# MarSaKi/ETPNav

Measured on AMD Instinct MI355X. Metric: planner fwd+bwd steps/sec at batch 32, 36-view x768 pano + 80-tok instr, higher is better.
Workload: dtype bf16

## Files before the change

### etpnav_amd/csrc/attn_rows.hip

```cpp
#include <stdlib.h>
#include <string.h>

#include "kernels.h"

namespace etp {
namespace {

constexpr int TQ = 128;
constexpr int TP = 144;
constexpr int PROJ_K = 768;
constexpr int PROJ_SLAB_K = 128;
constexpr int PROJ_RING = 3;
#ifndef ETP_PROJ_FETCH_AT
#define ETP_PROJ_FETCH_AT 2
#endif
__device__ __forceinline__ int tile_off(int row, int chunk) { return row * TQ + ((chunk ^ (row & 7)) << 4); }

struct RowArgs {
  const bf16_t *Q, *K, *V; long ldq, ldk, ldv;
  float* lse;
  bf16_t* ctx; long ldc;
  int nh, Lq, Lk;
  Drop drop;
  const uint8_t* keymask; int mask_mode; const float* dist; const float* sp_w; const float* sp_b;
  float alpha;
  const bf16_t* dO; long ldd;
  bf16_t *dQ, *dK, *dV; long lddq, lddk, lddv;
  float *d_sp_w, *d_sp_b;
  const bf16_t* W; long ldw; int Kp;
  const bf16_t* X; long ldx; const float* bqkv;
  int kv_mod;
};

__device__ __forceinline__ f32x4_t mma32(const uint4& a, const uint4& b, f32x4_t c) {
  return __builtin_amdgcn_mfma_f32_16x16x32_bf16(__builtin_bit_cast(bf16x8_t, a), __builtin_bit_cast(bf16x8_t, b), c, 0, 0, 0);
}
__device__ __forceinline__ f32x4_t mma16(const short4_t& a, const short4_t& b, f32x4_t c) {
  return __builtin_amdgcn_mfma_f32_16x16x16bf16_1k(a, b, c, 0, 0, 0);
}
__device__ __forceinline__ short4_t pack4(float a, float b, float c, float d) {
  const uint2 u = make_uint2(pack_bf16(a, b), pack_bf16(c, d));
  return __builtin_bit_cast(short4_t, u);
}
__device__ __forceinline__ uint4 frag(const char* tile, int row0, int s, int lane) {
  return *reinterpret_cast<const uint4*>(tile + tile_off(row0 + (lane & 15), s * 4 + (lane >> 4)));
}
__device__ __forceinline__ short4_t frag_t4(const char* tile, int row0, int col0, int lane) {
  const int i = lane & 15, g = lane >> 4;
  const int col = col0 + (i & 3) * 4;
  const char* p = tile + tile_off(row0 + 4 * g + (i >> 2), col >> 3) + (col & 7) * 2;
  typedef short4_t __attribute__((address_space(3))) * lds_s4;
  return __builtin_amdgcn_ds_read_tr16_b64_v4i16((lds_s4)(p));
}

template <int MAXROWS> struct TileRegs {
  static constexpr int N = (MAXROWS * 8 + 255) / 256;
  uint4 v[N];
};
template <int MAXROWS>
__device__ __forceinline__ void tile_fetch(TileRegs<MAXROWS>& r, const bf16_t* __restrict__ g, long ld, int rows_valid, int rows_pad,
                                           int tid, int nthr) {
#pragma unroll
  for (int j = 0; j < TileRegs<MAXROWS>::N; ++j) {
    const int q = tid + j * nthr, row = q >> 3, c = (q & 7) * 8;
    uint4 v = make_uint4(0u, 0u, 0u, 0u);
    if (row < rows_pad) {
      const bool ok = row < rows_valid;
      v = *reinterpret_cast<const uint4*>(g + (long)min(row, rows_valid - 1) * ld + c);
      v.x = ok ? v.x : 0u; v.y = ok ? v.y : 0u; v.z = ok ? v.z : 0u; v.w = ok ? v.w : 0u;
    }
    r.v[j] = v;
  }
}
template <int MAXROWS>
__device__ __forceinline__ void tile_commit(char* lds, const TileRegs<MAXROWS>& r, int rows_pad, int tid, int nthr) {
#pragma unroll
  for (int j = 0; j < TileRegs<MAXROWS>::N; ++j) {
    const int q = tid + j * nthr, row = q >> 3;
    if (row < rows_pad) *reinterpret_cast<uint4*>(lds + tile_off(row, q & 7)) = r.v[j];
  }
}

__device__ __forceinline__ void store_rows16(char* strip, const f32x4_t (&acc)[4], float scale, bf16_t* __restrict__ g0, long ld,
                                             int rows_valid, int lane) {
  const int i = lane & 15, g = lane >> 4;
#pragma unroll
  for (int t = 0; t < 4; ++t)
    *reinterpret_cast<uint2*>(strip + i * TP + (16 * t + 4 * g) * 2) =
        make_uint2(pack_bf16(acc[t][0] * scale, acc[t][1] * scale), pack_bf16(acc[t][2] * scale, acc[t][3] * scale));
  __builtin_amdgcn_wave_barrier();
#pragma unroll
  for (int j = 0; j < 2; ++j) {
    const int c = lane + 64 * j, row = c >> 3, part = c & 7;
    const uint4 v = *reinterpret_cast<const uint4*>(strip + row * TP + part * 16);
    if (row < rows_valid) *reinterpret_cast<uint4*>(g0 + (long)row * ld + part * 8) = v;
  }
  __builtin_amdgcn_wave_barrier();
}

template <int WN>
__device__ __forceinline__ void proj_load_w(uint4 (&w)[WN], const bf16_t* __restrict__ Wg, long ldw, int s, int tid, int nthr) {
#pragma unroll
  for (int j = 0; j < WN; ++j) {
    const int p = tid + j * nthr;
    w[j] = make_uint4(0u, 0u, 0u, 0u);
    if (p < PROJ_SLAB_K * 8) w[j] = *reinterpret_cast<const uint4*>(Wg + (long)(s * PROJ_SLAB_K + (p >> 3)) * ldw + (p & 7) * 8);
  }
}
__device__ __forceinline__ void proj_load_y(uint4 (&y)[4], const bf16_t* __restrict__ Yr, int s, bool computing, bool qok) {
#pragma unroll
  for (int u = 0; u < 4; ++u) {
    uint4 v = make_uint4(0u, 0u, 0u, 0u);
    if (computing) v = *reinterpret_cast<const uint4*>(Yr + s * PROJ_SLAB_K + 32 * u);
    v.x = qok ? v.x : 0u; v.y = qok ? v.y : 0u; v.z = qok ? v.z : 0u; v.w = qok ? v.w : 0u;
    y[u] = v;
  }
}
template <int WN>
__device__ __forceinline__ void proj_commit_w(char* slab, const uint4 (&w)[WN], int tid, int nthr) {
#pragma unroll
  for (int j = 0; j < WN; ++j) {
    const int p = tid + j * nthr, kk = p >> 3;
    const int row = (kk & ~0x1c) | ((kk & 0x4) << 2) | ((kk & 0x18) >> 1);
    if (p < PROJ_SLAB_K * 8) *reinterpret_cast<uint4*>(slab + tile_off(row, p & 7)) = w[j];
  }
}

template <int WN>
__device__ __forceinline__ void qkv_load_w(uint4 (&w)[WN], const bf16_t* __restrict__ W, long ldw, int Hh, int h, int s, int tid, int nthr) {
#pragma unroll
  for (int j = 0; j < WN; ++j) {
    const int p = tid + j * nthr, row = p >> 3;
    w[j] = make_uint4(0u, 0u, 0u, 0u);
    if (p < 192 * 8) w[j] = *reinterpret_cast<const uint4*>(W + (long)((row >> 6) * Hh + h * 64 + (row & 63)) * ldw + s * 64 + (p & 7) * 8);
  }
}
__device__ __forceinline__ void qkv_load_x(uint4 (&y)[2], const bf16_t* __restrict__ Xr, int s, bool computing, bool ok) {
#pragma unroll
  for (int u = 0; u < 2; ++u) {
    uint4 v = make_uint4(0u, 0u, 0u, 0u);
    if (computing) v = *reinterpret_cast<const uint4*>(Xr + s * 64 + 32 * u);
    v.x = ok ? v.x : 0u; v.y = ok ? v.y : 0u; v.z = ok ? v.z : 0u; v.w = ok ? v.w : 0u;
    y[u] = v;
  }
}
template <int WN>
__device__ __forceinline__ void qkv_commit_w(char* slab, const uint4 (&w)[WN], int tid, int nthr) {
#pragma unroll
  for (int j = 0; j < WN; ++j) {
    const int p = tid + j * nthr;
    if (p < 192 * 8) *reinterpret_cast<uint4*>(slab + tile_off(p >> 3, p & 7)) = w[j];
  }
}

__device__ __forceinline__ float key_term(const uint8_t* km, int col, int Lk, int mask_mode) {
  if (col >= Lk) return -INFINITY;
  if (km && !km[col]) return mask_mode ? -INFINITY : -10000.0f;
  return 0.f;
}

constexpr int QKV_SLAB_K = 64;
constexpr int QKV_RING = 2;
constexpr int QKV_SLAB_BYTES = 192 * TQ;
__host__ __device__ constexpr int rows_fwd_bias_off(int BKV, int nwaves) {
  const int base = 2 * BKV * TQ + BKV * 4 + nwaves * 16 * TP, ring = QKV_RING * QKV_SLAB_BYTES;
  return base < ring ? ring : base;
}
__host__ __device__ constexpr int rows_fwd_lds(int BKV, int nwaves, bool qkv) {
  return qkv ? rows_fwd_bias_off(BKV, nwaves) + 192 * 4 : 2 * BKV * TQ + BKV * 4 + nwaves * 16 * TP;
}

template <int NKT, bool HAS_DIST, bool QKV>
__global__ __launch_bounds__(512) void rows_fwd_kernel(const RowArgs a) {
  constexpr int BKV = NKT * 16;
  extern __shared__ __attribute__((aligned(16))) char smem[];
  char* kt = smem; char* vt = smem + BKV * TQ;
  float* kadd = reinterpret_cast<float*>(smem + 2 * BKV * TQ);
  const int tid = threadIdx.x, nthr = blockDim.x, lane = tid & 63, wave = tid >> 6, i = lane & 15, g = lane >> 4;
  const int bh = blockIdx.x, b = bh / a.nh, h = bh % a.nh;
  char* strip = smem + 2 * BKV * TQ + BKV * 4 + wave * 16 * TP;
  const int q = wave * 16 + i, qc = min(q, a.Lq - 1);
  uint4 qf0, qf1;

  const int bk = a.kv_mod > 0 ? b % a.kv_mod : b;
  if constexpr (!QKV) {
    TileRegs<BKV> rk, rv;
    tile_fetch<BKV>(rk, a.K + (long)bk * a.Lk * a.ldk + h * 64, a.ldk, a.Lk, BKV, tid, nthr);
    tile_fetch<BKV>(rv, a.V + (long)bk * a.Lk * a.ldv + h * 64, a.ldv, a.Lk, BKV, tid, nthr);
    const bf16_t* Qr = a.Q + ((long)b * a.Lq + qc) * a.ldq + h * 64 + g * 8;
    qf0 = *reinterpret_cast<const uint4*>(Qr); qf1 = *reinterpret_cast<const uint4*>(Qr + 32);
    if (tid < BKV) kadd[tid] = key_term(a.keymask ? a.keymask + (long)bk * a.Lk : nullptr, tid, a.Lk, a.mask_mode);
    tile_commit<BKV>(kt, rk, BKV, tid, nthr);
    tile_commit<BKV>(vt, rv, BKV, tid, nthr);
  } else {
    constexpr int NS = PROJ_K / QKV_SLAB_K, WN = 6;
    const int Hh = a.nh * 64;
    float* bias_l = reinterpret_cast<float*>(smem + rows_fwd_bias_off(BKV, nthr >> 6));
    const bool computing = wave < NKT, tok_ok = q < a.Lq;
    const bf16_t* Xr = a.X + ((long)b * a.Lq + qc) * a.ldx + g * 8;
    uint4 wr[WN], yb[2][2];
    f32x4_t acc[12];
#pragma unroll
    for (int t = 0; t < 12; ++t) acc[t] = f32x4_t{0.f, 0.f, 0.f, 0.f};
    if (tid < 192) bias_l[tid] = a.bqkv ? a.bqkv[(tid >> 6) * Hh + h * 64 + (tid & 63)] : 0.f;
    qkv_load_w<WN>(wr, a.W, a.ldw, Hh, h, 0, tid, nthr); qkv_load_x(yb[0], Xr, 0, computing, tok_ok);
    qkv_commit_w<WN>(smem, wr, tid, nthr);
    __syncthreads();
#pragma unroll
    for (int s = 0; s < NS; ++s) {
      if (s + 1 < NS) { qkv_load_w<WN>(wr, a.W, a.ldw, Hh, h, s + 1, tid, nthr); qkv_load_x(yb[(s + 1) & 1], Xr, s + 1, computing, tok_ok); }
      if (computing) {
        const char* slab = smem + (s & 1) * QKV_SLAB_BYTES;
#pragma unroll
        for (int u = 0; u < 2; ++u)
#pragma unroll
          for (int t = 0; t < 12; ++t) acc[t] = mma32(frag(slab, 16 * t, u, lane), yb[s & 1][u], acc[t]);
      }
      if (s + 1 < NS) qkv_commit_w<WN>(smem + ((s + 1) & 1) * QKV_SLAB_BYTES, wr, tid, nthr);
      __syncthreads();
    }
    if (tid < BKV) kadd[tid] = key_term(a.keymask ? a.keymask + (long)b * a.Lk : nullptr, tid, a.Lk, a.mask_mode);
    if (computing) {
      const int rows_valid = a.Lq - wave * 16;
#pragma unroll
      for (int sec = 0; sec < 3; ++sec) {
#pragma unroll
        for (int t = 0; t < 4; ++t) {
          const float4 bb = *reinterpret_cast<const float4*>(bias_l + sec * 64 + 16 * t + 4 * g);
          const f32x4_t c = acc[sec * 4 + t];
          *reinterpret_cast<uint2*>(strip + i * TP + (16 * t + 4 * g) * 2) =
              make_uint2(pack_bf16(c[0] + bb.x, c[1] + bb.y), pack_bf16(c[2] + bb.z, c[3] + bb.w));
        }
        __builtin_amdgcn_wave_barrier();
        if (sec == 0) {
          qf0 = *reinterpret_cast<const uint4*>(strip + i * TP + g * 16);
          qf1 = *reinterpret_cast<const uint4*>(strip + i * TP + 64 + g * 16);
        }
        bf16_t* dst = const_cast<bf16_t*>(sec == 0 ? a.Q : sec == 1 ? a.K : a.V);
        const long ld = sec == 0 ? a.ldq : sec == 1 ? a.ldk : a.ldv;
        char* tile = sec == 1 ? kt : vt;
#pragma unroll
        for (int j = 0; j < 2; ++j) {
          const int c = lane + 64 * j, row = c >> 3, part = c & 7;
          uint4 v = *reinterpret_cast<const uint4*>(strip + row * TP + part * 16);
          if (row < rows_valid) *reinterpret_cast<uint4*>(dst + ((long)b * a.Lq + wave * 16 + row) * ld + h * 64 + part * 8) = v;
          else v = make_uint4(0u, 0u, 0u, 0u);
          if (sec > 0) *reinterpret_cast<uint4*>(tile + tile_off(wave * 16 + row, part)) = v;
        }
        __builtin_amdgcn_wave_barrier();
      }
    }
  }
  __syncthreads();
  if (wave * 16 >= a.Lq) return;

  f32x4_t s[NKT];
#pragma unroll
  for (int n = 0; n < NKT; ++n) {
    s[n] = f32x4_t{0.f, 0.f, 0.f, 0.f};
    s[n] = mma32(frag(kt, 16 * n, 0, lane), qf0, s[n]);
    s[n] = mma32(frag(kt, 16 * n, 1, lane), qf1, s[n]);
  }
  float w = 0.f, b0 = 0.f;
  const float* drow = nullptr;
  if constexpr (HAS_DIST) { w = a.sp_w[0]; b0 = a.sp_b[0]; drow = a.dist + ((long)b * a.Lq + qc) * a.Lk; }
  float mx = -INFINITY;
#pragma unroll
  for (int n = 0; n < NKT; ++n) {
    const float4 ka4 = *reinterpret_cast<const float4*>(kadd + 16 * n + 4 * g);
    const float ka[4] = {ka4.x, ka4.y, ka4.z, ka4.w};
#pragma unroll
    for (int r = 0; r < 4; ++r) {
      float v = s[n][r] * a.alpha + ka[r];
      if constexpr (HAS_DIST) {
        const int key = 16 * n + 4 * g + r;
        if (key < a.Lk) v += w * drow[key] + b0;
      }
      s[n][r] = v;
      mx = fmaxf(mx, v);
    }
  }
  mx = fmaxf(mx, __shfl_xor(mx, 16, 64));
  mx = fmaxf(mx, __shfl_xor(mx, 32, 64));
  float sum = 0.f;
#pragma unroll
  for (int n = 0; n < NKT; ++n)
#pragma unroll
    for (int r = 0; r < 4; ++r) {
      const float e = __expf(s[n][r] - mx);
      s[n][r] = e;
      sum += e;
    }
  sum += __shfl_xor(sum, 16, 64);
  sum += __shfl_xor(sum, 32, 64);
  const float inv = 1.0f / sum;
  if (g == 0 && q < a.Lq) a.lse[(long)bh * a.Lq + q] = mx + __logf(sum);

  short4_t pb[NKT];
  const bool dropping = a.drop.p > 0.f;
  const uint32_t rbase = ((uint32_t)bh * a.Lq + q) * (uint32_t)a.Lk;
#pragma unroll
  for (int n = 0; n < NKT; ++n) {
    float p[4];
#pragma unroll
    for (int r = 0; r < 4; ++r) p[r] = s[n][r] * inv;
    if (dropping) {
      float dm[4];
      drop_mult_run<4>(a.drop.seed, rbase + 16 * n + 4 * g, a.drop.p, a.drop.inv_keep, dm);
#pragma unroll
      for (int r = 0; r < 4; ++r) p[r] *= dm[r];
    }
    pb[n] = pack4(p[0], p[1], p[2], p[3]);
  }
  f32x4_t o[4];
#pragma unroll
  for (int t = 0; t < 4; ++t) o[t] = f32x4_t{0.f, 0.f, 0.f, 0.f};
#pragma unroll
  for (int n = 0; n < NKT; ++n)
#pragma unroll
    for (int t = 0; t < 4; ++t) o[t] = mma16(frag_t4(vt, 16 * n, 16 * t, lane), pb[n], o[t]);
  store_rows16(strip, o, 1.0f, a.ctx + ((long)b * a.Lq + wave * 16) * a.ldc + h * 64, a.ldc, a.Lq - wave * 16, lane);
}

struct BwdLds {
  int q, d, k, v, kadd, lse, D, red, strip, ring, total;
  __host__ __device__ BwdLds(int BQ, int BKV, bool proj = false) {
    d = 0; q = BQ * TQ; k = 2 * BQ * TQ; v = k + BKV * TQ; kadd = v + BKV * TQ;
    lse = kadd + BKV * 4; D = lse + 128 * 4; red = D + 128 * 4; strip = red + 16 * 4; total = strip + 8 * 16 * TP;
    ring = BQ * TQ;
    if (proj && total < ring + PROJ_RING * PROJ_SLAB_K * TQ) total = ring + PROJ_RING * PROJ_SLAB_K * TQ;
  }
};

template <int NKT, bool HAS_DIST, bool PROJ>
__global__ __launch_bounds__(512) void rows_bwd_kernel(const RowArgs a) {
  constexpr int BKV = NKT * 16;
  extern __shared__ __attribute__((aligned(16))) char smem[];
  const int nqt = (a.Lq + 15) >> 4, BQ = nqt * 16;
  const BwdLds L(BQ, BKV, PROJ);
  char *qt = smem + L.q, *dt = smem + L.d, *kt = smem + L.k, *vt = smem + L.v;
  float* kadd = reinterpret_cast<float*>(smem + L.kadd);
  float* lse = reinterpret_cast<float*>(smem + L.lse);
  float* Dl = reinterpret_cast<float*>(smem + L.D);
  float* red = reinterpret_cast<float*>(smem + L.red);
  const int tid = threadIdx.x, nthr = blockDim.x, lane = tid & 63, wave = tid >> 6, i = lane & 15, g = lane >> 4;
  const int bh = blockIdx.x, b = bh / a.nh, h = bh % a.nh;
  const bool dropping = a.drop.p > 0.f;
  char* strip = smem + L.strip + wave * 16 * TP;

  {
    TileRegs<128> rq, rd;
    TileRegs<BKV> rk, rv;
    const int bk = a.kv_mod > 0 ? b % a.kv_mod : b;
#define FETCH_QKV()                                                                                        \
    tile_fetch<128>(rq, a.Q + (long)b * a.Lq * a.ldq + h * 64, a.ldq, a.Lq, BQ, tid, nthr);                 \
    tile_fetch<BKV>(rk, a.K + (long)bk * a.Lk * a.ldk + h * 64, a.ldk, a.Lk, BKV, tid, nthr);               \
    tile_fetch<BKV>(rv, a.V + (long)bk * a.Lk * a.ldv + h * 64, a.ldv, a.Lk, BKV, tid, nthr)
    if constexpr (!PROJ) {
      FETCH_QKV();
      tile_fetch<128>(rd, a.dO + (long)b * a.Lq * a.ldd + h * 64, a.ldd, a.Lq, BQ, tid, nthr);
    } else {
      constexpr int SLAB = PROJ_SLAB_K * TQ, WN = 4, NS = PROJ_K / PROJ_SLAB_K;
      char* ring = smem + L.ring;
      const bf16_t* Wg = a.W + h * 64;
      const int qrow = wave * 16 + i;
      const bool computing = wave < nqt, qok = qrow < a.Lq;
      const bf16_t* Yr = a.dO + ((long)b * a.Lq + min(qrow, a.Lq - 1)) * a.ldd + g * 8;
      uint4 wr[2][WN], yb[3][4];
      f32x4_t acc[4];
#pragma unroll
      for (int t = 0; t < 4; ++t) acc[t] = f32x4_t{0.f, 0.f, 0.f, 0.f};
      proj_load_w<WN>(wr[0], Wg, a.ldw, 0, tid, nthr); proj_load_y(yb[0], Yr, 0, computing, qok);
      proj_load_w<WN>(wr[1], Wg, a.ldw, 1, tid, nthr); proj_load_y(yb[1], Yr, 1, computing, qok);
      proj_commit_w<WN>(ring, wr[0], tid, nthr);
      __syncthreads();
#pragma unroll
      for (int s = 0; s < NS; ++s) {
        if (s + 2 < NS) { proj_load_w<WN>(wr[s % 2], Wg, a.ldw, s + 2, tid, nthr); proj_load_y(yb[(s + 2) % 3], Yr, s + 2, computing, qok); }
        if (s + ETP_PROJ_FETCH_AT == NS) { FETCH_QKV(); }
        if (computing) {
          const char* slab = ring + (s % 3) * SLAB;
#pragma unroll
          for (int u = 0; u < 4; ++u)
#pragma unroll
            for (int t = 0; t < 4; ++t) {
              const short4_t lo = frag_t4(slab, 32 * u, 16 * t, lane), hi = frag_t4(slab, 32 * u + 16, 16 * t, lane);
              const uint2 l2 = __builtin_bit_cast(uint2, lo), h2 = __builtin_bit_cast(uint2, hi);
              acc[t] = mma32(make_uint4(l2.x, l2.y, h2.x, h2.y), yb[s % 3][u], acc[t]);
            }
        }
        if (s + 1 < NS) {
          proj_commit_w<WN>(ring + ((s + 1) % 3) * SLAB, wr[(s + 1) % 2], tid, nthr);
          __syncthreads();
        }
      }
      if (computing) {
#pragma unroll
        for (int t = 0; t < 4; ++t)
          *reinterpret_cast<uint2*>(dt + tile_off(16 * wave + i, 2 * t + (g >> 1)) + (g & 1) * 8) =
              make_uint2(pack_bf16(acc[t][0], acc[t][1]), pack_bf16(acc[t][2], acc[t][3]));
      }
      __syncthreads();
    }
#undef FETCH_QKV
    if (tid < BKV) kadd[tid] = key_term(a.keymask ? a.keymask + (long)bk * a.Lk : nullptr, tid, a.Lk, a.mask_mode);
    if (tid < 128) lse[tid] = tid < a.Lq ? a.lse[(long)bh * a.Lq + tid] : INFINITY;
    tile_commit<128>(qt, rq, BQ, tid, nthr);
    if constexpr (!PROJ) tile_commit<128>(dt, rd, BQ, tid, nthr);
    tile_commit<BKV>(kt, rk, BKV, tid, nthr);
    tile_commit<BKV>(vt, rv, BKV, tid, nthr);
  }
  float w = 0.f, b0 = 0.f;
  if constexpr (HAS_DIST) { w = a.sp_w[0]; b0 = a.sp_b[0]; }
  __syncthreads();

  float aw = 0.f, ab = 0.f;
  if (wave < nqt) {
    const int q = wave * 16 + i;
    const bool qok = q < a.Lq;
    const uint4 qf0 = frag(qt, 16 * wave, 0, lane), qf1 = frag(qt, 16 * wave, 1, lane);
    const uint4 df0 = frag(dt, 16 * wave, 0, lane), df1 = frag(dt, 16 * wave, 1, lane);
    const float lse_i = lse[q];
    const float* drow = HAS_DIST ? a.dist + ((long)b * a.Lq + min(q, a.Lq - 1)) * a.Lk : nullptr;
    const uint32_t rbase = ((uint32_t)bh * a.Lq + q) * (uint32_t)a.Lk;
    f32x4_t p[NKT], dp[NKT];
    float dv4[NKT][4];
    float Dp = 0.f;
#pragma unroll
    for (int n = 0; n < NKT; ++n) {
      f32x4_t st = f32x4_t{0.f, 0.f, 0.f, 0.f}, dpt = f32x4_t{0.f, 0.f, 0.f, 0.f};
      st = mma32(frag(kt, 16 * n, 0, lane), qf0, st);
      st = mma32(frag(kt, 16 * n, 1, lane), qf1, st);
      dpt = mma32(frag(vt, 16 * n, 0, lane), df0, dpt);
      dpt = mma32(frag(vt, 16 * n, 1, lane), df1, dpt);
      const float4 ka4 = *reinterpret_cast<const float4*>(kadd + 16 * n + 4 * g);
      const float ka[4] = {ka4.x, ka4.y, ka4.z, ka4.w};
      float dm[4] = {1.f, 1.f, 1.f, 1.f};
      if (dropping) drop_mult_run<4>(a.drop.seed, rbase + 16 * n + 4 * g, a.drop.p, a.drop.inv_keep, dm);
#pragma unroll
      for (int r = 0; r < 4; ++r) {
        const int key = 16 * n + 4 * g + r;
        float v = st[r] * a.alpha + ka[r];
        if constexpr (HAS_DIST) {
          const float dd = (qok && key < a.Lk) ? drow[key] : 0.f;
          dv4[n][r] = dd;
          if (key < a.Lk) v += w * dd + b0;
        }
        const float pe = __expf(v - lse_i);
        const float dpv = dpt[r] * dm[r];
        p[n][r] = pe; dp[n][r] = dpv;
        Dp += pe * dpv;
      }
    }
    Dp += __shfl_xor(Dp, 16, 64);
    Dp += __shfl_xor(Dp, 32, 64);
    if (g == 0) Dl[q] = Dp;
    short4_t dsb[NKT];
#pragma unroll
    for (int n = 0; n < NKT; ++n) {
      float ds[4];
#pragma unroll
      for (int r = 0; r < 4; ++r) {
        ds[r] = p[n][r] * (dp[n][r] - Dp);
        if constexpr (HAS_DIST) { aw += ds[r] * dv4[n][r]; ab += ds[r]; }
      }
      dsb[n] = pack4(ds[0], ds[1], ds[2], ds[3]);
    }
    f32x4_t dq[4];
#pragma unroll
    for (int t = 0; t < 4; ++t) dq[t] = f32x4_t{0.f, 0.f, 0.f, 0.f};
#pragma unroll
    for (int n = 0; n < NKT; ++n)
#pragma unroll
      for (int t = 0; t < 4; ++t) dq[t] = mma16(frag_t4(kt, 16 * n, 16 * t, lane), dsb[n], dq[t]);
    store_rows16(strip, dq, a.alpha, a.dQ + ((long)b * a.Lq + wave * 16) * a.lddq + h * 64, a.lddq, a.Lq - wave * 16, lane);
  }
  if constexpr (HAS_DIST) {
    aw = wave_sum(aw); ab = wave_sum(ab);
    if (lane == 0) { red[wave] = aw; red[8 + wave] = ab; }
  }
  __syncthreads();
  if constexpr (HAS_DIST) {
    if (tid == 0 && a.d_sp_w != nullptr) {
      float sw = 0.f, sb = 0.f;
      for (int k = 0; k < (nthr >> 6); ++k) { sw += red[k]; sb += red[8 + k]; }
      atomicAdd(a.d_sp_w, sw);
      atomicAdd(a.d_sp_b, sb);
    }
  }

  if (wave * 16 < a.Lk) {
    const int key = wave * 16 + i;
    const bool kok = key < a.Lk;
    const uint4 kf0 = frag(kt, 16 * wave, 0, lane), kf1 = frag(kt, 16 * wave, 1, lane);
    const uint4 vf0 = frag(vt, 16 * wave, 0, lane), vf1 = frag(vt, 16 * wave, 1, lane);
    const float ka = kadd[key];
    f32x4_t dv[4], dk[4];
#pragma unroll
    for (int t = 0; t < 4; ++t) { dv[t] = f32x4_t{0.f, 0.f, 0.f, 0.f}; dk[t] = f32x4_t{0.f, 0.f, 0.f, 0.f}; }
    for (int m = 0; m < nqt; ++m) {
      f32x4_t s = f32x4_t{0.f, 0.f, 0.f, 0.f}, dpm = f32x4_t{0.f, 0.f, 0.f, 0.f};
      s = mma32(frag(qt, 16 * m, 0, lane), kf0, s);
      s = mma32(frag(qt, 16 * m, 1, lane), kf1, s);
      dpm = mma32(frag(dt, 16 * m, 0, lane), vf0, dpm);
      dpm = mma32(frag(dt, 16 * m, 1, lane), vf1, dpm);
      const float4 l4 = *reinterpret_cast<const float4*>(lse + 16 * m + 4 * g);
      const float4 D4 = *reinterpret_cast<const float4*>(Dl + 16 * m + 4 * g);
      const float lr[4] = {l4.x, l4.y, l4.z, l4.w}, Dr[4] = {D4.x, D4.y, D4.z, D4.w};
      float pd[4], ds[4];
#pragma unroll
      for (int r = 0; r < 4; ++r) {
        const int qq = 16 * m + 4 * g + r;
        float v = s[r] * a.alpha + ka;
        if constexpr (HAS_DIST) {
          if (kok && qq < a.Lq) v += w * a.dist[((long)b * a.Lq + qq) * a.Lk + key] + b0;
        }
        const float pe = __expf(v - lr[r]);
        float mult = 1.0f;
        if (dropping) mult = drop_mult(a.drop.seed, ((uint32_t)bh * a.Lq + qq) * (uint32_t)a.Lk + key, a.drop.p, a.drop.inv_keep);
        pd[r] = pe * mult;
        ds[r] = pe * (dpm[r] * mult - Dr[r]);
      }
      const short4_t pb = pack4(pd[0], pd[1], pd[2], pd[3]), dsb = pack4(ds[0], ds[1], ds[2], ds[3]);
#pragma unroll
      for (int t = 0; t < 4; ++t) {
        dv[t] = mma16(frag_t4(dt, 16 * m, 16 * t, lane), pb, dv[t]);
        dk[t] = mma16(frag_t4(qt, 16 * m, 16 * t, lane), dsb, dk[t]);
      }
    }
    store_rows16(strip, dv, 1.0f, a.dV + ((long)b * a.Lk + wave * 16) * a.lddv + h * 64, a.lddv, a.Lk - wave * 16, lane);
    store_rows16(strip, dk, a.alpha, a.dK + ((long)b * a.Lk + wave * 16) * a.lddk + h * 64, a.lddk, a.Lk - wave * 16, lane);
  }
}

template <int NKT, bool HAS_DIST, bool QKV> int launch_rows_fwd_q(const RowArgs& k, int blocks, int threads, hipStream_t st) {
  const int smem = rows_fwd_lds(NKT * 16, threads / 64, QKV);
  auto kern = rows_fwd_kernel<NKT, HAS_DIST, QKV>;
  if (smem > 64 * 1024) ETP_CHECK_HIP(ensure_dyn_lds(reinterpret_cast<const void*>(kern), smem));
  ETP_LAUNCH_ROW(ROWF_ATTN_FWD, kern, dim3(blocks), dim3(threads), smem, st, k);
  ETP_CHECK_LAUNCH(QKV ? "attn_rows_fwd_qkv" : "attn_rows_fwd");
  return ETP_OK;
}
template <int NKT, bool HAS_DIST> int launch_rows_fwd(const RowArgs& k, int blocks, int threads, hipStream_t st) {
  return k.X ? launch_rows_fwd_q<NKT, HAS_DIST, true>(k, blocks, threads, st) : launch_rows_fwd_q<NKT, HAS_DIST, false>(k, blocks, threads, st);
}
template <int NKT, bool HAS_DIST, bool PROJ> int launch_rows_bwd_p(const RowArgs& k, int blocks, int threads, hipStream_t st) {
  const BwdLds L(((k.Lq + 15) >> 4) * 16, NKT * 16, PROJ);
  auto kern = rows_bwd_kernel<NKT, HAS_DIST, PROJ>;
  ETP_CHECK_HIP(ensure_dyn_lds(reinterpret_cast<const void*>(kern), BwdLds(128, NKT * 16, PROJ).total));
  ETP_LAUNCH_ROW(ROWF_ATTN_BWD, kern, dim3(blocks), dim3(threads), L.total, st, k);
  ETP_CHECK_LAUNCH(PROJ ? "attn_rows_bwd_proj" : "attn_rows_bwd");
  return ETP_OK;
}
template <int NKT, bool HAS_DIST> int launch_rows_bwd(const RowArgs& k, int blocks, int threads, hipStream_t st) {
  return k.W ? launch_rows_bwd_p<NKT, HAS_DIST, true>(k, blocks, threads, st) : launch_rows_bwd_p<NKT, HAS_DIST, false>(k, blocks, threads, st);
}

template <bool HAS_DIST> int dispatch_fwd(int nkt, const RowArgs& k, int blocks, int threads, hipStream_t st) {
  switch (nkt) {
    case 1: return launch_rows_fwd<1, HAS_DIST>(k, blocks, threads, st);
    case 2: return launch_rows_fwd<2, HAS_DIST>(k, blocks, threads, st);
    case 3: return launch_rows_fwd<3, HAS_DIST>(k, blocks, threads, st);
    case 4: return launch_rows_fwd<4, HAS_DIST>(k, blocks, threads, st);
    case 5: return launch_rows_fwd<5, HAS_DIST>(k, blocks, threads, st);
    case 6: return launch_rows_fwd<6, HAS_DIST>(k, blocks, threads, st);
    case 7: return launch_rows_fwd<7, HAS_DIST>(k, blocks, threads, st);
    default: return launch_rows_fwd<8, HAS_DIST>(k, blocks, threads, st);
  }
}
template <bool HAS_DIST> int dispatch_bwd(int nkt, const RowArgs& k, int blocks, int threads, hipStream_t st) {
  switch (nkt) {
    case 1: return launch_rows_bwd<1, HAS_DIST>(k, blocks, threads, st);
    case 2: return launch_rows_bwd<2, HAS_DIST>(k, blocks, threads, st);
    case 3: return launch_rows_bwd<3, HAS_DIST>(k, blocks, threads, st);
    case 4: return launch_rows_bwd<4, HAS_DIST>(k, blocks, threads, st);
    case 5: return launch_rows_bwd<5, HAS_DIST>(k, blocks, threads, st);
    case 6: return launch_rows_bwd<6, HAS_DIST>(k, blocks, threads, st);
    case 7: return launch_rows_bwd<7, HAS_DIST>(k, blocks, threads, st);
    default: return launch_rows_bwd<8, HAS_DIST>(k, blocks, threads, st);
  }
}

RowArgs make_row_args(int nh, const AttnBuf& a, void* P, float alpha, Drop drop) {
  RowArgs k;
  memset(&k, 0, sizeof(k));
  k.Q = (const bf16_t*)a.Q; k.K = (const bf16_t*)a.K; k.V = (const bf16_t*)a.V; k.ldq = a.ldq; k.ldk = a.ldk; k.ldv = a.ldv;
  k.lse = (float*)P; k.nh = nh; k.Lq = a.Lq; k.Lk = a.Lk; k.drop = drop;
  k.keymask = a.keymask; k.mask_mode = a.mask_mode; k.dist = a.dist; k.sp_w = a.sp_w; k.sp_b = a.sp_b; k.alpha = alpha;
  k.kv_mod = a.kv_mod;
  return k;
}

}

bool attn_rows_ok(int dt, const AttnBuf& a, long ldc) {
  const bool on = opt_on(OPT_ATTN_ROWS, true);
  if (!on || dt != ETP_BF16) return false;
  if (a.Lq > 128 || a.Lk > 128 || a.Lq < 1 || a.Lk < 1 || a.ldS < 2) return false;
// ... 62 lines not shown
```

### etpnav_amd/csrc/planner.hip

```cpp
#include <string.h>

#include <algorithm>
#include <functional>
#include <vector>

#include "kernels.h"

namespace etp {

struct AttnP { int qkv_w, qkv_b, o_w, o_b, ln_g, ln_b; };
struct FfnP { int i_w, i_b, o_w, o_b, ln_g, ln_b; };
struct TxtLayerP { AttnP att; FfnP ffn; };
struct PanoLayerP { int in_w, in_b, out_w, out_b, l1_w, l1_b, l2_w, l2_b, n1_g, n1_b, n2_g, n2_b; };
struct XLayerP { int q_w, q_b, kv_w, kv_b, xo_w, xo_b, xln_g, xln_b; AttnP self; FfnP ffn;
                 AttnP lself; FfnP lffn; };

struct PInfo { std::string name; int ndim; long shape[2]; int region; long offset; long numel; };

}

struct etp_planner {
  etp_config cfg;
  std::vector<etp::PInfo> params;
  long total = 0, n_matrix = 0;
// ... 388 lines not shown
  g.M = a.Lq; g.N = a.Lk; g.K = dh; g.nb_inner = nh; g.alpha = alpha;
  ETP_TRY(launch_gemm(dt, dt, 0, 0, g, a.B * nh, st));
  ETP_TRY(softmax_fwd(dt, P, a.keymask, a.dist, a.sp_w, a.sp_b, a.B, nh, a.Lq, a.Lk, a.ldS, a.mask_mode, st));
  const void* Pv = P;
  if (drop.p > 0.f) {
    ETP_TRY(drop_rows(dt, P, a.Pd, (long)a.B * nh * a.Lq, a.Lk, a.ldS, drop, st));
    Pv = a.Pd;
  }
  GemmArgs h = base_args();
  h.A = Pv; h.lda = a.ldS; h.sAo = g.sCo; h.sAi = g.sCi;
  h.B = a.V; h.ldb = a.ldv; h.sBo = (long)a.Lk * a.ldv; h.sBi = dh;
  h.C = ctx; h.ldc = ldc; h.sCo = (long)a.Lq * ldc; h.sCi = dh;
  h.M = a.Lq; h.N = dh; h.K = a.Lk; h.nb_inner = nh;
  return launch_gemm(dt, dt, 0, 1, h, a.B * nh, st);
}

int attn_bwd_impl(int dt, int nh, const AttnBuf& a, const void* P, const void* dctx, long ldd, void* dP, void* dQ, long lddq,
                  void* dK, long lddk, void* dV, long lddv, float alpha, float* d_sp_w, float* d_sp_b, hipStream_t st,
                  Drop drop) {
  const int dh = 64;
  ETP_REQUIRE(!a.dkv_sum || a.kv_mod > 0, "summed dK/dV (AttnBuf::dkv_sum) needs per-episode K/V indirection (kv_mod > 0)");
  {
    const int epc = dt == ETP_BF16 ? 8 : 4;
    const long ldc_f = a.O != nullptr ? a.ldo : ldd;
    const bool dal = lddq % epc == 0 && lddk % epc == 0 && lddv % epc == 0;
    const int fam = attn_family(dt, a, ldc_f);
    if (fam == ATTN_FAMILY_ROWS) {
      ETP_REQUIRE(ldd % 8 == 0 && dal, "the forward of this shape kept lse only (register-resident kernels): the backward needs "
                                       "16-byte-aligned dctx / dQ / dK / dV rows");
      return attn_rows_bwd(nh, a, P, dctx, ldd, dQ, lddq, dK, lddk, dV, lddv, alpha, d_sp_w, d_sp_b, st, drop);
    }
    ETP_REQUIRE(a.kv_mod == 0 || fam == ATTN_FAMILY_FLASH, "per-episode K/V indirection (AttnBuf::kv_mod) needs the register-resident or the streaming attention kernels (bf16, no distance bias)");
    if (fam == ATTN_FAMILY_TILE) {
      if (attn_fused_ok(dt, a, ldd) && dal)
        return attn_fused_bwd(dt, nh, a, P, dctx, ldd, dQ, lddq, dK, lddk, dV, lddv, alpha, d_sp_w, d_sp_b, st, drop);
    } else if (fam == ATTN_FAMILY_FLASH) {
      ETP_REQUIRE(a.O != nullptr && a.ldo % epc == 0 && ldd % epc == 0 && dal,
                  "the forward of this shape kept lse only (streaming kernels): the backward needs the forward output (ctx) and "
                  "16-byte-aligned dctx / dQ / dK / dV rows");
      return attn_flash_bwd(nh, a, P, dctx, ldd, dQ, lddq, dK, lddk, dV, lddv, alpha, st, drop);
    }
  }
  ETP_REQUIRE(drop.p == 0.f || a.Pd, "attention dropout on the unfused path needs the second probability buffer (AttnBuf::Pd)");
  const long sPo = (long)nh * a.Lq * a.ldS, sPi = (long)a.Lq * a.ldS;
  GemmArgs g = base_args();
  g.A = dctx; g.lda = ldd; g.sAo = (long)a.Lq * ldd; g.sAi = dh;
  g.B = a.V; g.ldb = a.ldv; g.sBo = (long)a.Lk * a.ldv; g.sBi = dh;
  g.C = dP; g.ldc = a.ldS; g.sCo = sPo; g.sCi = sPi;
  g.M = a.Lq; g.N = a.Lk; g.K = dh; g.nb_inner = nh;
  ETP_TRY(launch_gemm(dt, dt, 0, 0, g, a.B * nh, st));
  if (drop.p > 0.f) ETP_TRY(drop_rows(dt, dP, dP, (long)a.B * nh * a.Lq, a.Lk, a.ldS, drop, st));
  GemmArgs v = base_args();
  v.A = drop.p > 0.f ? a.Pd : P; v.lda = a.ldS; v.sAo = sPo; v.sAi = sPi;
  v.B = dctx; v.ldb = ldd; v.sBo = (long)a.Lq * ldd; v.sBi = dh;
  v.C = dV; v.ldc = lddv; v.sCo = (long)a.Lk * lddv; v.sCi = dh;
  v.M = a.Lk; v.N = dh; v.K = a.Lq; v.nb_inner = nh;
  ETP_TRY(launch_gemm(dt, dt, 1, 1, v, a.B * nh, st));
  ETP_TRY(softmax_bwd(dt, P, dP, a.dist, d_sp_w, d_sp_b, a.B, nh, a.Lq, a.Lk, a.ldS, st));
  GemmArgs q = base_args();
  q.A = dP; q.lda = a.ldS; q.sAo = sPo; q.sAi = sPi;
  q.B = a.K; q.ldb = a.ldk; q.sBo = (long)a.Lk * a.ldk; q.sBi = dh;
  q.C = dQ; q.ldc = lddq; q.sCo = (long)a.Lq * lddq; q.sCi = dh;
  q.M = a.Lq; q.N = dh; q.K = a.Lk; q.nb_inner = nh; q.alpha = alpha;
  ETP_TRY(launch_gemm(dt, dt, 0, 1, q, a.B * nh, st));
  GemmArgs k = base_args();
  k.A = dP; k.lda = a.ldS; k.sAo = sPo; k.sAi = sPi;
  k.B = a.Q; k.ldb = a.ldq; k.sBo = (long)a.Lq * a.ldq; k.sBi = dh;
  k.C = dK; k.ldc = lddk; k.sCo = (long)a.Lk * lddk; k.sCi = dh;
  k.M = a.Lk; k.N = dh; k.K = a.Lq; k.nb_inner = nh; k.alpha = alpha;
  return launch_gemm(dt, dt, 1, 1, k, a.B * nh, st);
}

static bool fold_projection(Opt o, int workgroups, bool by_grid) {
  const char* s = opt_str(o);
  if (s) return s[0] != '0';
  return by_grid && workgroups <= cu_count();
}

static int attn_bwd_proj(const Ctx& c, const AttnBuf& a, const void* P, const void* dy, int wi, void* dctx, int M, void* dP, void* dQ,
                         long lddq, void* dK, long lddk, void* dV, long lddv, float* d_sp_w, float* d_sp_b, Drop drop) {
  const int H = c.H;
  const void* W = c.pl->pw(wi);
  const int epc = 8;
  const bool four_waves = a.Lq <= 64 && a.Lk <= 64;
  if (c.dt == ETP_BF16 && (fold_projection(OPT_ATTN_PROJ, a.B * c.nh, true) || (four_waves && fold_projection(OPT_ATTN_PROJ, 0, true))) &&
      attn_rows_ok(c.dt, a, H) && attn_rows_proj_ok(H, W, H) &&
      lddq % epc == 0 && lddk % epc == 0 && lddv % epc == 0)
    return attn_rows_bwd(c.nh, a, P, dy, H, dQ, lddq, dK, lddk, dV, lddv, 0.125f, d_sp_w, d_sp_b, c.st, drop, W, H, H);
  ETP_TRY(linear_dgrad(c, dy, H, wi, dctx, H, M, H, H, ETP_ACT_NONE, nullptr, 0, nullptr, 0));
  return attn_bwd_impl(c.dt, c.nh, a, P, dctx, H, dP, dQ, lddq, dK, lddk, dV, lddv, 0.125f, d_sp_w, d_sp_b, c.st, drop);
}

static int attn_fwd_qkv(const Ctx& c, const AttnBuf& a, void* P, void* ctx, const void* x, int wi, int bi, void* qkv, int M, Drop drop) {
  const int H = c.H;
  const void* W = c.pl->pw(wi);
  if (c.dt == ETP_BF16 && fold_projection(OPT_ATTN_QKV, a.B * c.nh, false) && attn_rows_ok(c.dt, a, H) && attn_rows_qkv_ok(c.nh, a, x, H, W, H))
    return attn_rows_fwd(c.nh, a, P, ctx, H, 0.125f, c.st, drop, x, H, W, H, bi >= 0 ? c.pl->pf(bi) : nullptr);
  ETP_TRY(linear_fwd(c, x, H, wi, bi, qkv, 3 * H, M, 3 * H, H, ETP_ACT_NONE, nullptr, nullptr, 0));
  return attn_fwd_impl(c.dt, c.nh, a, P, ctx, H, 0.125f, c.st, drop);
}

struct Act { float* f; void* t; };
static Act take_act(Bump& b, int dt, long n) {
  Act a;
  a.f = (float*)b.take((size_t)n * 4);
  a.t = dt == ETP_BF16 ? b.take((size_t)n * 2) : (void*)a.f;
  return a;
}
static inline void* lp(const Act& a, int dt) { return dt == ETP_BF16 ? a.t : nullptr; }
static Act take_act2(Bump& b, int dt, long n) {
  Act a;
  a.f = (float*)b.take((size_t)n * 4);
  a.t = b.take((size_t)n * dtype_size(dt));
  return a;
}
static inline void* lp2(const Ctx& c, const Act& a, const Drop& d) { return (c.dt == ETP_BF16 || d.p > 0.f) ? a.t : nullptr; }
static inline const void* op2(const Ctx& c, const Act& a, const Drop& d) { return (c.dt == ETP_BF16 || d.p > 0.f) ? a.t : (void*)a.f; }

struct SelfAttStash { void *qkv, *P, *ctx; float* s; float* st; Act y; void* Pd; };
struct FfnStash { void *z, *h; float* s; float* st; Act y; };
struct CrossStash { void *q, *kv, *P, *ctx; float* s; float* st; Act y; void* Pd; };

static SelfAttStash plan_self(Bump& b, int dt, long M, int Bn, int nh, int L, int ldS, int H) {
  const size_t es = dtype_size(dt);
  SelfAttStash s;
  s.qkv = b.take(M * 3 * H * es);
  s.P = b.take((size_t)Bn * nh * L * ldS * es);
  s.ctx = b.take(M * H * es);
  s.s = (float*)b.take(M * H * 4);
  s.st = (float*)b.take(M * 2 * sizeof(float));
  s.y = take_act(b, dt, M * H);
  s.Pd = attn_needs_unfused(dt, L, L) ? b.take((size_t)Bn * nh * L * ldS * es) : nullptr;
  return s;
}
static FfnStash plan_ffn(Bump& b, int dt, long M, int H, int I) {
  const size_t es = dtype_size(dt);
  FfnStash f;
  f.z = b.take(M * I * es);
  f.h = b.take(M * I * es);
  f.s = (float*)b.take(M * H * 4);
  f.st = (float*)b.take(M * 2 * sizeof(float));
  f.y = take_act(b, dt, M * H);
  return f;
}

struct BwdWs { Act t1; void *t2, *dI, *dqkv, *dP; float* lnp; };
static BwdWs plan_ws(Bump& b, int dt, long M, int Bn, int nh, int Lq, int ldS, int H, int I) {
  const size_t es = dtype_size(dt);
  BwdWs w;
  w.t1 = take_act2(b, dt, M * H);
  w.t2 = b.take(M * H * es);
  w.dI = b.take(M * I * es);
  w.dqkv = b.take(M * 3 * H * es);
  w.dP = b.take((size_t)Bn * nh * Lq * ldS * es);
  w.lnp = (float*)b.take(ln_bwd_part_bytes((int)M, H));
  return w;
}

static int ln_bwd_chain(const Ctx& c, const float* dy, const float* x, const float* stats, int gi, int bi, const float* add,
                        float* dx, void* dxt, int M, const Drop& d, float* part) {
  etp_planner* pl = c.pl;
  const bool two_stage = opt_on(OPT_LNBWD_TWO_STAGE, true);
  if (!two_stage) part = nullptr;
  ETP_TRY(ln_bwd_s(c.dt, dy, x, stats, pl->pf(gi), add, dx, dxt, pl->gf(gi), pl->gf(bi), M, c.H, c.st, d, part));
  if (!part) return ETP_OK;
  float* dg = pl->gf(gi); float* db = pl->gf(bi);
  const int H = c.H;
  hipStream_t sw = c.sw;
// ... 1082 lines not shown
```

Before: 256.7.

## Stream projection weight slabs via global_load_lds and hoist dist loads

The fused backward output-projection path now streams weight slabs straight into an LDS ring with global_load_lds_dwordx4 issued by four loader waves. This replaces the register staging and LDS commit, and synchronisation uses vmcnt/lgkmcnt waits plus raw s_barrier. Tile fetches become unconditional clamped loads, with zero-masking moved to the LDS commit. Distance-bias loads in forward and backward are hoisted ahead of the MMA work and use branchless selects. The host also enables the fused projection backward whenever Lq<=64 regardless of Lk, which routes more layers through this kernel; the hand-written asm and wait counts risk ordering mistakes.

```diff
diff --git a/etpnav_amd/csrc/attn_rows.hip b/etpnav_amd/csrc/attn_rows.hip
--- a/etpnav_amd/csrc/attn_rows.hip
+++ b/etpnav_amd/csrc/attn_rows.hip
@@ -11,9 +11,6 @@
 constexpr int PROJ_K = 768;
 constexpr int PROJ_SLAB_K = 128;
 constexpr int PROJ_RING = 3;
-#ifndef ETP_PROJ_FETCH_AT
-#define ETP_PROJ_FETCH_AT 2
-#endif
 __device__ __forceinline__ int tile_off(int row, int chunk) { return row * TQ + ((chunk ^ (row & 7)) << 4); }
 
 struct RowArgs {
@@ -58,26 +55,22 @@
   uint4 v[N];
 };
 template <int MAXROWS>
-__device__ __forceinline__ void tile_fetch(TileRegs<MAXROWS>& r, const bf16_t* __restrict__ g, long ld, int rows_valid, int rows_pad,
-                                           int tid, int nthr) {
+__device__ __forceinline__ void tile_fetch(TileRegs<MAXROWS>& r, const bf16_t* __restrict__ g, long ld, int rows_valid, int tid, int nthr) {
 #pragma unroll
   for (int j = 0; j < TileRegs<MAXROWS>::N; ++j) {
     const int q = tid + j * nthr, row = q >> 3, c = (q & 7) * 8;
-    uint4 v = make_uint4(0u, 0u, 0u, 0u);
-    if (row < rows_pad) {
-      const bool ok = row < rows_valid;
-      v = *reinterpret_cast<const uint4*>(g + (long)min(row, rows_valid - 1) * ld + c);
-      v.x = ok ? v.x : 0u; v.y = ok ? v.y : 0u; v.z = ok ? v.z : 0u; v.w = ok ? v.w : 0u;
-    }
-    r.v[j] = v;
+    r.v[j] = *reinterpret_cast<const uint4*>(g + (long)min(row, rows_valid - 1) * ld + c);
   }
 }
 template <int MAXROWS>
-__device__ __forceinline__ void tile_commit(char* lds, const TileRegs<MAXROWS>& r, int rows_pad, int tid, int nthr) {
+__device__ __forceinline__ void tile_commit(char* lds, const TileRegs<MAXROWS>& r, int rows_valid, int rows_pad, int tid, int nthr) {
 #pragma unroll
   for (int j = 0; j < TileRegs<MAXROWS>::N; ++j) {
     const int q = tid + j * nthr, row = q >> 3;
-    if (row < rows_pad) *reinterpret_cast<uint4*>(lds + tile_off(row, q & 7)) = r.v[j];
+    const bool ok = row < rows_valid;
+    uint4 v = r.v[j];
+    v.x = ok ? v.x : 0u; v.y = ok ? v.y : 0u; v.z = ok ? v.z : 0u; v.w = ok ? v.w : 0u;
+    if (row < rows_pad) *reinterpret_cast<uint4*>(lds + tile_off(row, q & 7)) = v;
   }
 }
 
@@ -98,32 +91,20 @@
   __builtin_amdgcn_wave_barrier();
 }
 
-template <int WN>
-__device__ __forceinline__ void proj_load_w(uint4 (&w)[WN], const bf16_t* __restrict__ Wg, long ldw, int s, int tid, int nthr) {
-#pragma unroll
-  for (int j = 0; j < WN; ++j) {
-    const int p = tid + j * nthr;
-    w[j] = make_uint4(0u, 0u, 0u, 0u);
-    if (p < PROJ_SLAB_K * 8) w[j] = *reinterpret_cast<const uint4*>(Wg + (long)(s * PROJ_SLAB_K + (p >> 3)) * ldw + (p & 7) * 8);
-  }
-}
-__device__ __forceinline__ void proj_load_y(uint4 (&y)[4], const bf16_t* __restrict__ Yr, int s, bool computing, bool qok) {
-#pragma unroll
-  for (int u = 0; u < 4; ++u) {
-    uint4 v = make_uint4(0u, 0u, 0u, 0u);
-    if (computing) v = *reinterpret_cast<const uint4*>(Yr + s * PROJ_SLAB_K + 32 * u);
-    v.x = qok ? v.x : 0u; v.y = qok ? v.y : 0u; v.z = qok ? v.z : 0u; v.w = qok ? v.w : 0u;
-    y[u] = v;
-  }
-}
-template <int WN>
-__device__ __forceinline__ void proj_commit_w(char* slab, const uint4 (&w)[WN], int tid, int nthr) {
-#pragma unroll
-  for (int j = 0; j < WN; ++j) {
-    const int p = tid + j * nthr, kk = p >> 3;
-    const int row = (kk & ~0x1c) | ((kk & 0x4) << 2) | ((kk & 0x18) >> 1);
-    if (p < PROJ_SLAB_K * 8) *reinterpret_cast<uint4*>(slab + tile_off(row, p & 7)) = w[j];
-  }
+__device__ __forceinline__ void proj_glds(unsigned voff, const char* sbase, unsigned lds_addr) {
+  asm volatile(
+      "s_mov_b32 m0, %2\n\t"
+      "s_nop 0\n\t"
+      "global_load_lds_dwordx4 %0, %1"
+      :
+      : "v"(voff), "s"(sbase), "s"(lds_addr)
+      : "memory");
+}
+template <int N> __device__ __forceinline__ void proj_wait_vm() { asm volatile("s_waitcnt vmcnt(%0)" ::"n"(N) : "memory"); }
+__device__ __forceinline__ void proj_wait_lgkm0() { asm volatile("s_waitcnt lgkmcnt(0)" ::: "memory"); }
+__device__ __forceinline__ void proj_load_y(uint4 (&y)[4], const bf16_t* __restrict__ Yr, int s) {
+#pragma unroll
+  for (int u = 0; u < 4; ++u) y[u] = *reinterpret_cast<const uint4*>(Yr + s * PROJ_SLAB_K + 32 * u);
 }
 
 template <int WN>
@@ -185,13 +166,13 @@
   const int bk = a.kv_mod > 0 ? b % a.kv_mod : b;
   if constexpr (!QKV) {
     TileRegs<BKV> rk, rv;
-    tile_fetch<BKV>(rk, a.K + (long)bk * a.Lk * a.ldk + h * 64, a.ldk, a.Lk, BKV, tid, nthr);
-    tile_fetch<BKV>(rv, a.V + (long)bk * a.Lk * a.ldv + h * 64, a.ldv, a.Lk, BKV, tid, nthr);
+    tile_fetch<BKV>(rk, a.K + (long)bk * a.Lk * a.ldk + h * 64, a.ldk, a.Lk, tid, nthr);
+    tile_fetch<BKV>(rv, a.V + (long)bk * a.Lk * a.ldv + h * 64, a.ldv, a.Lk, tid, nthr);
     const bf16_t* Qr = a.Q + ((long)b * a.Lq + qc) * a.ldq + h * 64 + g * 8;
     qf0 = *reinterpret_cast<const uint4*>(Qr); qf1 = *reinterpret_cast<const uint4*>(Qr + 32);
     if (tid < BKV) kadd[tid] = key_term(a.keymask ? a.keymask + (long)bk * a.Lk : nullptr, tid, a.Lk, a.mask_mode);
-    tile_commit<BKV>(kt, rk, BKV, tid, nthr);
-    tile_commit<BKV>(vt, rv, BKV, tid, nthr);
+    tile_commit<BKV>(kt, rk, a.Lk, BKV, tid, nthr);
+    tile_commit<BKV>(vt, rv, a.Lk, BKV, tid, nthr);
   } else {
     constexpr int NS = PROJ_K / QKV_SLAB_K, WN = 6;
     const int Hh = a.nh * 64;
@@ -254,6 +235,16 @@
   __syncthreads();
   if (wave * 16 >= a.Lq) return;
 
+  float w = 0.f, b0 = 0.f;
+  float dd[HAS_DIST ? NKT : 1][4];
+  if constexpr (HAS_DIST) {
+    w = a.sp_w[0]; b0 = a.sp_b[0];
+    const float* drow = a.dist + ((long)b * a.Lq + qc) * a.Lk;
+#pragma unroll
+    for (int n = 0; n < NKT; ++n)
+#pragma unroll
+      for (int r = 0; r < 4; ++r) dd[n][r] = drow[min(16 * n + 4 * g + r, a.Lk - 1)];
+  }
   f32x4_t s[NKT];
 #pragma unroll
   for (int n = 0; n < NKT; ++n) {
@@ -261,9 +252,6 @@
     s[n] = mma32(frag(kt, 16 * n, 0, lane), qf0, s[n]);
     s[n] = mma32(frag(kt, 16 * n, 1, lane), qf1, s[n]);
   }
-  float w = 0.f, b0 = 0.f;
-  const float* drow = nullptr;
-  if constexpr (HAS_DIST) { w = a.sp_w[0]; b0 = a.sp_b[0]; drow = a.dist + ((long)b * a.Lq + qc) * a.Lk; }
   float mx = -INFINITY;
 #pragma unroll
   for (int n = 0; n < NKT; ++n) {
@@ -274,7 +262,8 @@
       float v = s[n][r] * a.alpha + ka[r];
       if constexpr (HAS_DIST) {
         const int key = 16 * n + 4 * g + r;
-        if (key < a.Lk) v += w * drow[key] + b0;
+        const float vb = v + (w * dd[n][r] + b0);
+        v = key < a.Lk ? vb : v;
       }
       s[n][r] = v;
       mx = fmaxf(mx, v);
@@ -353,62 +342,86 @@
     TileRegs<BKV> rk, rv;
     const int bk = a.kv_mod > 0 ? b % a.kv_mod : b;
 #define FETCH_QKV()                                                                                        \
-    tile_fetch<128>(rq, a.Q + (long)b * a.Lq * a.ldq + h * 64, a.ldq, a.Lq, BQ, tid, nthr);                 \
-    tile_fetch<BKV>(rk, a.K + (long)bk * a.Lk * a.ldk + h * 64, a.ldk, a.Lk, BKV, tid, nthr);               \
-    tile_fetch<BKV>(rv, a.V + (long)bk * a.Lk * a.ldv + h * 64, a.ldv, a.Lk, BKV, tid, nthr)
+    tile_fetch<128>(rq, a.Q + (long)b * a.Lq * a.ldq + h * 64, a.ldq, a.Lq, tid, nthr);                     \
+    tile_fetch<BKV>(rk, a.K + (long)bk * a.Lk * a.ldk + h * 64, a.ldk, a.Lk, tid, nthr);                    \
+    tile_fetch<BKV>(rv, a.V + (long)bk * a.Lk * a.ldv + h * 64, a.ldv, a.Lk, tid, nthr)
     if constexpr (!PROJ) {
       FETCH_QKV();
-      tile_fetch<128>(rd, a.dO + (long)b * a.Lq * a.ldd + h * 64, a.ldd, a.Lq, BQ, tid, nthr);
+      tile_fetch<128>(rd, a.dO + (long)b * a.Lq * a.ldd + h * 64, a.ldd, a.Lq, tid, nthr);
     } else {
-      constexpr int SLAB = PROJ_SLAB_K * TQ, WN = 4, NS = PROJ_K / PROJ_SLAB_K;
+      constexpr int SLAB = PROJ_SLAB_K * TQ, NS = PROJ_K / PROJ_SLAB_K, NP = 4;
       char* ring = smem + L.ring;
-      const bf16_t* Wg = a.W + h * 64;
-      const int qrow = wave * 16 + i;
-      const bool computing = wave < nqt, qok = qrow < a.Lq;
+      const int wv = __builtin_amdgcn_readfirstlane(wave);
+      const bool computing = wv < nqt, loader = wv < 4;
+      const int qrow = wv * 16 + i;
+      const bool qok = qrow < a.Lq;
       const bf16_t* Yr = a.dO + ((long)b * a.Lq + min(qrow, a.Lq - 1)) * a.ldd + g * 8;
-      uint4 wr[2][WN], yb[3][4];
+      const int r5 = 8 * (wv & 3) + (lane >> 3);
+      const int kk = (r5 & 3) | ((r5 & 0x10) >> 2) | ((r5 & 0xc) << 1);
+      const unsigned voff = (unsigned)(((long)kk * a.ldw + (((lane & 7) ^ (r5 & 7)) << 3)) * 2);
+      const char* wbase = reinterpret_cast<const char*>(a.W + h * 64);
+      const long piece_stride = 32 * a.ldw * 2, slab_stride = (long)PROJ_SLAB_K * a.ldw * 2;
+      const unsigned piece0 = (unsigned)(uintptr_t)((__attribute__((address_space(3))) char*)ring) + (unsigned)(wv & 3) * 1024u;
+      auto issue_slab = [&](int s) {
+        if (loader) {
+#pragma unroll
+          for (int c = 0; c < NP; ++c) proj_glds(voff, wbase + s * slab_stride + c * piece_stride, piece0 + (unsigned)((s % PROJ_RING) * SLAB + c * 4096));
+        }
+      };
+      uint4 yb[2][4];
       f32x4_t acc[4];
 #pragma unroll
       for (int t = 0; t < 4; ++t) acc[t] = f32x4_t{0.f, 0.f, 0.f, 0.f};
-      proj_load_w<WN>(wr[0], Wg, a.ldw, 0, tid, nthr); proj_load_y(yb[0], Yr, 0, computing, qok);
-      proj_load_w<WN>(wr[1], Wg, a.ldw, 1, tid, nthr); proj_load_y(yb[1], Yr, 1, computing, qok);
-      proj_commit_w<WN>(ring, wr[0], tid, nthr);
-      __syncthreads();
+      proj_load_y(yb[0], Yr, 0);
+      proj_load_y(yb[1], Yr, 1);
+      __builtin_amdgcn_sched_barrier(0);
+#pragma unroll
+      for (int s = 0; s < PROJ_RING; ++s) issue_slab(s);
+      __builtin_amdgcn_sched_barrier(0);
+      if (loader) proj_wait_vm<2 * NP>(); else proj_wait_vm<0>();
+      __builtin_amdgcn_s_barrier();
+      __builtin_amdgcn_sched_barrier(0);
 #pragma unroll
       for (int s = 0; s < NS; ++s) {
-        if (s + 2 < NS) { proj_load_w<WN>(wr[s % 2], Wg, a.ldw, s + 2, tid, nthr); proj_load_y(yb[(s + 2) % 3], Yr, s + 2, computing, qok); }
-        if (s + ETP_PROJ_FETCH_AT == NS) { FETCH_QKV(); }
+        if (s >= 1 && s + 1 < NS) proj_load_y(yb[(s + 1) & 1], Yr, s + 1);
+        __builtin_amdgcn_sched_barrier(0);
+        if (s >= 1 && s + 2 < NS) issue_slab(s + 2);
+        __builtin_amdgcn_sched_barrier(0);
+        if (s + 1 == NS) { FETCH_QKV(); }
         if (computing) {
-          const char* slab = ring + (s % 3) * SLAB;
+          const char* slab = ring + (s % PROJ_RING) * SLAB;
 #pragma unroll
           for (int u = 0; u < 4; ++u)
 #pragma unroll
             for (int t = 0; t < 4; ++t) {
               const short4_t lo = frag_t4(slab, 32 * u, 16 * t, lane), hi = frag_t4(slab, 32 * u + 16, 16 * t, lane);
               const uint2 l2 = __builtin_bit_cast(uint2, lo), h2 = __builtin_bit_cast(uint2, hi);
-              acc[t] = mma32(make_uint4(l2.x, l2.y, h2.x, h2.y), yb[s % 3][u], acc[t]);
+              acc[t] = mma32(make_uint4(l2.x, l2.y, h2.x, h2.y), yb[s & 1][u], acc[t]);
             }
         }
         if (s + 1 < NS) {
-          proj_commit_w<WN>(ring + ((s + 1) % 3) * SLAB, wr[(s + 1) % 2], tid, nthr);
-          __syncthreads();
+          __builtin_amdgcn_sched_barrier(0);
+          if (loader && s + 2 < NS) proj_wait_vm<NP>(); else proj_wait_vm<0>();
+          proj_wait_lgkm0();
+          __builtin_amdgcn_s_barrier();
+          __builtin_amdgcn_sched_barrier(0);
         }
       }
       if (computing) {
 #pragma unroll
         for (int t = 0; t < 4; ++t)
-          *reinterpret_cast<uint2*>(dt + tile_off(16 * wave + i, 2 * t + (g >> 1)) + (g & 1) * 8) =
-              make_uint2(pack_bf16(acc[t][0], acc[t][1]), pack_bf16(acc[t][2], acc[t][3]));
+          *reinterpret_cast<uint2*>(dt + tile_off(16 * wv + i, 2 * t + (g >> 1)) + (g & 1) * 8) =
+              qok ? make_uint2(pack_bf16(acc[t][0], acc[t][1]), pack_bf16(acc[t][2], acc[t][3])) : make_uint2(0u, 0u);
       }
       __syncthreads();
     }
 #undef FETCH_QKV
     if (tid < BKV) kadd[tid] = key_term(a.keymask ? a.keymask + (long)bk * a.Lk : nullptr, tid, a.Lk, a.mask_mode);
     if (tid < 128) lse[tid] = tid < a.Lq ? a.lse[(long)bh * a.Lq + tid] : INFINITY;
-    tile_commit<128>(qt, rq, BQ, tid, nthr);
-    if constexpr (!PROJ) tile_commit<128>(dt, rd, BQ, tid, nthr);
-    tile_commit<BKV>(kt, rk, BKV, tid, nthr);
-    tile_commit<BKV>(vt, rv, BKV, tid, nthr);
+    tile_commit<128>(qt, rq, a.Lq, BQ, tid, nthr);
+    if constexpr (!PROJ) tile_commit<128>(dt, rd, a.Lq, BQ, tid, nthr);
+    tile_commit<BKV>(kt, rk, a.Lk, BKV, tid, nthr);
+    tile_commit<BKV>(vt, rv, a.Lk, BKV, tid, nthr);
   }
   float w = 0.f, b0 = 0.f;
   if constexpr (HAS_DIST) { w = a.sp_w[0]; b0 = a.sp_b[0]; }
@@ -508,12 +521,18 @@
       const float4 D4 = *reinterpret_cast<const float4*>(Dl + 16 * m + 4 * g);
       const float lr[4] = {l4.x, l4.y, l4.z, l4.w}, Dr[4] = {D4.x, D4.y, D4.z, D4.w};
       float pd[4], ds[4];
+      float dd[4] = {0.f, 0.f, 0.f, 0.f};
+      if constexpr (HAS_DIST) {
+#pragma unroll
+        for (int r = 0; r < 4; ++r) dd[r] = a.dist[((long)b * a.Lq + min(16 * m + 4 * g + r, a.Lq - 1)) * a.Lk + min(key, a.Lk - 1)];
+      }
 #pragma unroll
       for (int r = 0; r < 4; ++r) {
         const int qq = 16 * m + 4 * g + r;
         float v = s[r] * a.alpha + ka;
         if constexpr (HAS_DIST) {
-          if (kok && qq < a.Lq) v += w * a.dist[((long)b * a.Lq + qq) * a.Lk + key] + b0;
+          const float vb = v + (w * dd[r] + b0);
+          v = (kok && qq < a.Lq) ? vb : v;
         }
         const float pe = __expf(v - lr[r]);
         float mult = 1.0f;
diff --git a/etpnav_amd/csrc/planner.hip b/etpnav_amd/csrc/planner.hip
--- a/etpnav_amd/csrc/planner.hip
+++ b/etpnav_amd/csrc/planner.hip
@@ -494,8 +494,8 @@
   const int H = c.H;
   const void* W = c.pl->pw(wi);
   const int epc = 8;
-  const bool four_waves = a.Lq <= 64 && a.Lk <= 64;
-  if (c.dt == ETP_BF16 && (fold_projection(OPT_ATTN_PROJ, a.B * c.nh, true) || (four_waves && fold_projection(OPT_ATTN_PROJ, 0, true))) &&
+  const bool few_query_tiles = a.Lq <= 64;
+  if (c.dt == ETP_BF16 && (fold_projection(OPT_ATTN_PROJ, a.B * c.nh, true) || (few_query_tiles && fold_projection(OPT_ATTN_PROJ, 0, true))) &&
       attn_rows_ok(c.dt, a, H) && attn_rows_proj_ok(H, W, H) &&
       lddq % epc == 0 && lddk % epc == 0 && lddv % epc == 0)
     return attn_rows_bwd(c.nh, a, P, dy, H, dQ, lddq, dK, lddk, dV, lddv, 0.125f, d_sp_w, d_sp_b, c.st, drop, W, H, H);
```

After: 261.9 (median of 6 runs). 1.02x the previous value.
